# haowenz/chromap

Hardware: AMD Instinct MI355X
Metric: M paired reads mapped/s (ATAC preset, GRCh38 index) (higher is better)
Workload: dtype u64

## Files before the change

chromap_amd/csrc/cm_api.hip:

```cpp
#include <hip/hip_runtime.h>
#include <math.h>
#include <stdio.h>
#include <stdlib.h>
#include <string.h>

#include <string>
#include <vector>

#include "../../include/chromap_amd.h"
#include "cm_barcode_translate.h"
#include "cm_ctx.h"
#include "cm_kernels.h"
#include "cm_classes.h"
#include "cm_summary.h"
#include "cm_coop.h"
#include <chrono>
#include <mutex>
#include "cm_mapq_tables.h"

static thread_local std::string g_last_error;

static bool cm_debug_pool() { static const bool on = getenv("CM_DEBUG_POOL") != nullptr; return on; }
static thread_local std::string t_last_error;
void cm_set_error(cmgpu_ctx *ctx, const std::string &msg) {
// ... 68 lines not shown
    c->opt.exchange_overlap = value ? 1 : 0;
  } else if (n == "lanes") {
    if (value < 1 || value > 8) { cm_set_error(c, "lanes: 1..8"); return CMGPU_EINVAL; }
    c->opt.lanes = (int)value;
  } else if (n == "first_read_id") {
    if (value < 0 || value > 0xffffffffll) { cm_set_error(c, "first_read_id: 0..2^32-1"); return CMGPU_EINVAL; }
    c->first_read_id = (uint32_t)value;
  } else if (n == "heavy_mid_max") {
    c->opt.heavy_mid = (int)value;
  } else if (n == "heavy_last") {
    c->opt.heavy_last = (int)value;
  } else if (n == "probe_table_shift") {
    if (value < 0 || value > 4) { cm_set_error(c, "probe_table_shift: 0..4"); return CMGPU_EINVAL; }
    return cm_build_fast_table(c, (int)value);
  } else if (n == "long_read_fused") {
    c->opt.long_fused = value ? 1 : 0;
  } else if (n == "sam_format_group") {
    if (value != 8 && value != 16 && value != 64) { cm_set_error(c, "sam_format_group: 8, 16 or 64"); return CMGPU_EINVAL; }
    c->opt.sam_group = (int)value;
  } else if (n == "verify_planes") {
    c->opt.planes = value ? 1 : 0;
  } else if (n == "speculative_sizes") {
    c->opt.spec = value ? 1 : 0;
    if (value < 0) { c->cls_seen = 0; memset(c->cls_age, 0, sizeof(c->cls_age)); }
  } else if (n == "debug_candidate_capacity") {
    if (value > 0 && cm_ensure_candidate_arrays(c, (uint64_t)value)) { cm_set_error(c, "out of device memory (candidates)"); return CMGPU_ENOMEM; }
    c->pred_m_ok = value > 0; c->m_cap = (uint64_t)value; c->pred_n = 0xffffffffu;
  } else if (n == "coop_profile") {
    if (value) { if (c->coop_prof.ensure(64 * 8)) return CMGPU_ENOMEM; CM_HIPCHECK(c, hipMemset(c->coop_prof.p, 0, 64 * 8)); } else c->coop_prof.release();
  } else if (n == "coop_run_table") {
    c->opt.coop_rb = (int)value;
  } else if (n == "coop") {
    c->opt.coop = (int)value;
  } else if (n == "generic_kernels") {
    c->opt.generic_kernels = value ? 1 : 0;
  } else if (n == "item_limit") {
    c->opt.item_limit = value > 0 ? (uint64_t)value : 0xfffffff0ull;
  } else {
    cm_set_error(c, "unknown option " + n);
    return CMGPU_EINVAL;
  }
  return CMGPU_OK;
}

extern "C" int cmgpu_get_option(const cmgpu_ctx *c, const char *name, int64_t *value) {
  if (!c || !name || !value) return CMGPU_EINVAL;
  const std::string n(name);
  if (n == "probe_lookups_per_lane") *value = c->opt.probe_variant & 15;
  else if (n == "probe_pair_prefetch") *value = (c->opt.probe_variant & 16) ? 1 : 0;
  else if (n == "mm_chunks") *value = c->opt.mm_chunks;
  else if (n == "h2d_copy_blocks") *value = c->opt.h2d_kernel;
  else if (n == "d2h_copy_blocks") *value = c->opt.d2h_kernel;
  else if (n == "prep_kernel") *value = c->opt.prep_kernel;
  else if (n == "prep_tile_reads") *value = c->opt.prep_tile_reads;
  else if (n == "item_limit") *value = (int64_t)c->opt.item_limit;
  else if (n == "lanes") *value = c->opt.lanes;
  else if (n == "coop") *value = c->opt.coop;
  else if (n == "generic_kernels") *value = c->opt.generic_kernels;
  else if (n == "alloc_us") *value = (int64_t)(c->alloc_seconds * 1e6);
  else if (n == "alloc_draw_us") *value = (int64_t)(c->alloc_draw_seconds * 1e6);
  else if (n.rfind("coop_profile_", 0) == 0) {
    const int k = atoi(n.c_str() + 13);
    unsigned long long v = 0;
    if (k < 0 || k > 63 || !c->coop_prof.p || hipMemcpy(&v, (const unsigned long long *)c->coop_prof.p + k, 8, hipMemcpyDeviceToHost) != hipSuccess) return CMGPU_EINVAL;
    *value = (int64_t)v;
  }
  else if (n == "probe_table_buckets") *value = c->fmask ? (int64_t)c->fmask + 1 : (int64_t)c->bmask + 1;
  else return CMGPU_EINVAL;
  return CMGPU_OK;
}

extern "C" const char *cmgpu_last_error(const cmgpu_ctx *ctx) { return ctx ? ctx->err.c_str() : g_last_error.c_str(); }

__global__ void k_repack(const uint32_t *__restrict__ flags, const uint64_t *__restrict__ keys,
                         const uint64_t *__restrict__ vals, uint64_t *__restrict__ bkt, uint32_t i0, uint32_t n) {
  const uint32_t j = blockIdx.x * 256 + threadIdx.x;
  if (j >= n) return;
  const uint32_t i = i0 + j;
  const uint32_t f = (flags[i >> 4] >> ((i & 0xfU) << 1)) & 3u;
  uint64_t k = keys[j], v = vals[j];
  if (f & 2u) { k = CM_EMPTY_KEY; v = 0; }
  else if (f & 1u) { k = CM_DELETED_KEY; v = 0; }
  bkt[2 * (uint64_t)i] = k;
  bkt[2 * (uint64_t)i + 1] = v;
}

__global__ __launch_bounds__(256) void k_rehash(const uint64_t *__restrict__ src, uint64_t n_src, uint64_t *__restrict__ dst, uint32_t mask) {
  const uint64_t i = (uint64_t)blockIdx.x * 256 + threadIdx.x;
  if (i >= n_src) return;
  const uint64_t key = src[2 * i], val = src[2 * i + 1];
  if (key == CM_EMPTY_KEY || key == CM_DELETED_KEY) return;
// ... 538 lines not shown
  d.goff = (const uint32_t *)c->goff.p; d.n_seq = c->n_seq;
  d.ref_pl = c->ref_pl_words && c->opt.planes ? (const CmPlRec *)c->ref_planes.p + CM_PL_LEAD : nullptr; d.ref_pl_words = c->ref_pl_words;
  d.p = c->p; d.p.single = c->single ? 1 : 0;
  d.mq.len_coef = (const double *)c->len_coef.p; d.mq.nsec_break = (const uint32_t *)c->nsec_break.p; d.mq.n_break = c->n_break;
  d.n_pairs = hi - lo; d.first_read_id = c->first_read_id + lo;
  d.rb0 = (const uint8_t *)c->rb0.p; d.rb1 = (const uint8_t *)c->rb1.p;
  d.ro0 = (const uint32_t *)c->ro0.p + lo; d.ro1 = (const uint32_t *)c->ro1.p + lo;
#define PTR(f, T) d.f = (T *)c->f.p;
  PTR(rlen, uint32_t) PTR(mm_cnt, uint32_t)
  PTR(mm_off, uint32_t) PTR(mm_hash, uint64_t) PTR(mm_ps, uint32_t) PTR(pr_val, uint64_t) PTR(pr_kind, uint8_t)
  PTR(hit_tot, uint32_t) PTR(hit_off, uint32_t) PTR(round2, uint8_t) PTR(rep_cnt, uint32_t) PTR(rep_len, uint32_t)
  PTR(hbuf, uint64_t) PTR(hcnt, uint8_t) PTR(n_pos_hit, uint32_t) PTR(ncp, uint32_t) PTR(ncn, uint32_t)
  PTR(aug, uint8_t) PTR(res_neg, int32_t) PTR(res_pos, int32_t) PTR(resc_n, uint32_t) PTR(resc_p, uint32_t)
  PTR(m_tot, uint32_t) PTR(m_off, uint32_t) PTR(mbuf, uint64_t) PTR(mcnt, uint8_t) PTR(mcp, uint32_t) PTR(mcn, uint32_t)
  PTR(force0, uint8_t) PTR(fbuf, uint64_t) PTR(fcnt, uint8_t) PTR(fcp, uint32_t) PTR(fcn, uint32_t) PTR(alive, uint8_t)
  PTR(dpos, uint64_t) PTR(derr, int16_t) PTR(dsplit, uint32_t) PTR(nv, uint32_t) PTR(v_off, uint32_t) PTR(v_err, int16_t) PTR(v_end, int16_t) PTR(ndp, uint32_t) PTR(ndn, uint32_t)
  PTR(min_err, int32_t) PTR(second_err, int32_t) PTR(n_best, int32_t) PTR(n_second, int32_t)
  PTR(pe_min, int32_t) PTR(pe_second, int32_t) PTR(pe_nbest, int32_t) PTR(pe_nsecond, int32_t)
  PTR(pe_first, uint32_t) PTR(pe_i1, uint32_t) PTR(pe_i2, uint32_t) PTR(pe_choice, uint32_t)
  PTR(stats, unsigned long long) PTR(srt_cnt, uint32_t) PTR(srt_list, uint32_t) PTR(hv_cnt, uint32_t) PTR(hv_list, uint32_t) PTR(rs_cnt, uint32_t) PTR(rs_list, uint32_t)
#undef PTR
  d.rec = (uint8_t *)c->rec.p + (size_t)lo * 24 * cm_rec_per_pair(c);
  d.rec_ok = (uint8_t *)c->rec_ok.p + (size_t)lo * cm_rec_per_pair(c);
  d.hv_stride = 2 * (hi - lo) + 1;
  d.perm_reads = c->use_perm ? (const uint32_t *)c->perm_reads.p : nullptr; d.perm_pairs = c->use_perm ? (const uint32_t *)c->perm_pairs.p : nullptr;
  d.coop_slab = (uint8_t *)c->coop_slab.p; d.coop_slab_cap = CM_SLAB_CAP; d.coop_slab_blocks = CM_SLAB_BLOCKS;
  d.cls_mask = c->cls_all || !c->opt.spec ? ~0ull : c->cls_seen;
  d.prof = (unsigned long long *)c->coop_prof.p;
  d.rs_pool = (uint64_t *)c->rs_pool.p; d.rs_pool_cap = c->rs_pool.p ? c->rs_pool_cap : 0u; d.rs_pool_off = (uint32_t *)c->rs_pool_off.p;
  d.abort = (const unsigned long long *)c->stats.p + CM_ST_ABORT;
  d.coop_rb = c->opt.coop_rb > 0 ? (uint32_t)c->opt.coop_rb : 0u;
  d.wq_dynamic = ((uint32_t)c->opt.coop >> 16) & 1u;
  d.generic_kernels = c->opt.generic_kernels ? 1u : 0u;
  if (c->has_rank) {
    d.rid_rank = (const uint32_t *)c->rid_rank.p;
    d.ref_off = (const uint64_t *)c->ref_off_r.p;
    d.ref_len = (const uint32_t *)c->ref_len_r.p;
  }
  if (c->has_pairs_rank) d.pairs_rank = (const uint32_t *)c->pairs_rank.p;
  if (c->has_barcodes) {
    d.bcb = (const uint8_t *)c->bcb.p; d.bcq = (const uint8_t *)c->bcq.p; d.bco = (const uint32_t *)c->bco.p + lo;
    d.wl = (const uint64_t *)c->wl.p; d.wl_mask = c->wl_mask; d.wl_num_sample = (double)c->wl_num_sample;
    d.pow10_tab = (const double *)c->pow10_tab.p;
    d.bc_key = c->bc_key.p ? (uint64_t *)c->bc_key.p + lo : nullptr; d.bc_ok = c->bc_ok.p ? (uint8_t *)c->bc_ok.p + lo : nullptr;
  }
}
static inline void mark(cmgpu_ctx *c, const char *name) {
  if (c->n_ev < CM_MAX_EVENTS) {
    (void)hipEventRecord(c->ev[c->n_ev], c->stream);
    c->ev_name[c->n_ev] = name;
    ++c->n_ev;
  }
}
static int scan_with_total(cmgpu_ctx *c, const uint32_t *in, uint32_t *out, uint32_t n, unsigned long long *total, bool wait = true) {
  hipStream_t s = c->stream;
  unsigned long long *acc = (unsigned long long *)c->stats.p + CM_ST_TOTAL;
  CM_HIPCHECK(c, hipMemsetAsync(acc, 0, 8, s));
  cm_launch_k_sum_u32(in, n, acc, s);
  cm_scan_u32(in, out, n, (uint32_t *)c->scan_tmp.p, s);
  CM_HIPCHECK(c, hipMemcpyAsync(total, acc, 8, hipMemcpyDeviceToHost, s));
  if (wait) CM_HIPCHECK(c, cm_stream_sync(s));
  return CMGPU_OK;
}
#define CM_RC_SPLIT (-100)
#define CM_RC_AGAIN_ALL_CLASSES (-101)
#define CM_RC_AGAIN_EXACT_SIZES (-102)
// ... 1202 lines not shown
```

chromap_amd/csrc/cm_ctx.h:

```cpp
#ifndef CM_CTX_H_
#define CM_CTX_H_
#include <hip/hip_runtime.h>

#include <string>
#include <thread>
#include <vector>

#include "../../include/chromap_amd.h"
#include "../../include/chromap_amd_debug.h"
#include "cm_types.h"

#define CM_MAX_EVENTS 32
#define CM_MAX_W_HOST 32

struct DevBuf {
  void *p = nullptr;
  size_t cap = 0;
  bool owned = true;
  int ensure(size_t bytes);
  void release();
};

struct CmTmpBuf : private DevBuf {
  using DevBuf::p;
// ... 67 lines not shown
  unsigned long long *h_matrix = nullptr;
  hipStream_t stream = nullptr;
  hipEvent_t ev_part = nullptr, ev_payload = nullptr;
  bool payload_pending = false;
  uint64_t sent_total = 0, recv_total = 0, steps = 0;
  uint64_t owned_by[64] = {};
};

#define CM_BATCH_SLOTS 8
struct CmBatchSlot {
  DevBuf rb0, rb1, ro0, ro1;
  uint32_t n_pairs = 0, first_read_id = 0, max_read_len = 1;
  size_t bases0 = 0, bases1 = 0;
};

struct CmOptions {
  int long_fused = 1;
  int planes = 1;
  int sam_group = 8;
  int d2h_kernel = 0;
  int h2d_kernel = 0;
  int probe_variant = 1;
  int mm_chunks = CM_MM_CHUNKS;
  int prep_tile_reads = 32;
  int prep_kernel = 0;
  uint64_t item_limit = 0xfffffff0ull;
  int exchange_overlap = 0;
  int s3b_cap = 0;
  int lanes = 1;
  int heavy_mid = 0;
  int heavy_max[3] = {0, 0, 0};
  int heavy_last = 0;
  int spec = 1;
  int generic_kernels = 0;
  int coop_rb = 0;
  int coop = 0xff;
};

struct cmgpu_ctx {
  CmOptions opt;
  int device = 0;
  hipStream_t stream = nullptr;
  hipStream_t stream2 = nullptr;
  hipStream_t stream_pack = nullptr;
  hipEvent_t chunk_ev[CM_MM_CHUNKS + 1] = {};
  std::string err;
  cmgpu_params hp;
  CmParams p;
  DevBuf bkt, occ, ref, ref_off, ref_len, len_coef, nsec_break;
  uint32_t bmask = 0, n_occ = 0, n_seq = 0;
  DevBuf bkt_fast, coop_prof;
  uint32_t fmask = 0;
  DevBuf ref_planes, read_planes;
  DevBuf mm_stage;
  uint64_t ref_pl_words = 0;
  int n_break = 0;
  uint64_t ref_bytes = 0;
  std::vector<uint64_t> h_ref_off;
  std::vector<uint32_t> h_ref_len;
  uint32_t n_pairs = 0, first_read_id = 0;
  size_t bases0 = 0, bases1 = 0;
  uint32_t max_read_len = 1;
  DevBuf rb0, rb1, ro0, ro1;
  DevBuf st_rb0, st_rb1, st_ro0, st_ro1, st_bcb, st_bcq, st_bco;
  DevBuf rlen, scratch_a, scratch_b , mm_cnt, mm_off, mm_hash, mm_ps, pr_val, pr_kind;
  DevBuf hit_tot, hit_off, round2, rep_cnt, rep_len, hbuf, hcnt, n_pos_hit, ncp, ncn;
// ... 155 lines not shown
```

chromap_amd/csrc/cm_kernels.hip:

```cpp
#include <hip/hip_runtime.h>
#include <stdio.h>
#include <string.h>
#include <cstring>
#include <atomic>
#include <map>
#include <mutex>
#include <type_traits>
#include <utility>
#include <rocprim/rocprim.hpp>

#include "cm_kernels.h"
#include "cm_stages.h"
#include "cm_classes.h"
#include "cm_coop.h"

#define CM_BLOCK 256

#define CM_ITEM_KERNEL(kname, fn, perm)                                      \
  __global__ __launch_bounds__(CM_BLOCK) void kname(CmDev d, uint32_t n) {   \
    if (d.abort && *d.abort) return;                                         \
    const uint32_t i = blockIdx.x * CM_BLOCK + threadIdx.x;                  \
    if (i < n) fn(d, d.perm ? d.perm[i] : i);                                \
  }

// ... 294 lines not shown
__global__ __launch_bounds__(CM_BLOCK) void k_s3a_count(CmDev d, uint32_t n) {
  const uint32_t i = blockIdx.x * CM_BLOCK + threadIdx.x;
  uint32_t tot = 0;
  if (i < n) {
    cm_s3a_count(d, i);
    tot = d.hit_tot[i];
  }
  const uint32_t cls = cm_hit_class(d, tot);
  __shared__ uint32_t sh_cnt[8], sh_base[8];
  if (threadIdx.x < 8) sh_cnt[threadIdx.x] = 0;
  __syncthreads();
  const uint32_t lane = threadIdx.x & 63u;
  const uint32_t ids[8] = {CM_L_HIT_WAVE, CM_L_HIT_B256A, CM_L_HIT_B256B, CM_L_HIT_SLAB, CM_L_HIT_G16, CM_L_HIT_B512, CM_L_HIT_WAVE_SMALL, CM_L_HIT_B1024};
  uint32_t slot = 0, mine = 8;
#pragma unroll
  for (uint32_t q = 0; q < 8; ++q) {
    const unsigned long long m = __ballot(cls == ids[q]);
    if (m == 0) continue;
    uint32_t base = 0;
    if (lane == (uint32_t)(__ffsll((long long)m) - 1)) base = atomicAdd(&sh_cnt[q], (uint32_t)__popcll(m));
    base = __shfl(base, __ffsll((long long)m) - 1, 64);
    if (cls == ids[q]) { slot = base + (uint32_t)__popcll(m & ((1ull << lane) - 1ull)); mine = q; }
  }
  __syncthreads();
  if (threadIdx.x < 8 && sh_cnt[threadIdx.x]) sh_base[threadIdx.x] = atomicAdd(cm_list_cnt(d, ids[threadIdx.x]), sh_cnt[threadIdx.x]);
  __syncthreads();
  if (mine < 8) cm_list(d, ids[mine])[sh_base[mine] + slot] = i;
}
__global__ __launch_bounds__(CM_BLOCK) void k_s3b_candidates(CmDev d, uint32_t n, uint32_t cap) {
  uint64_t *sh_h = reinterpret_cast<uint64_t *>(cm_lds);
  uint8_t *sh_c = cm_lds + (size_t)cap * blockDim.x * 8;
  const uint32_t i = blockIdx.x * blockDim.x + threadIdx.x;
  if (i < n && d.hit_tot[i] <= cap) cm_s3b_candidates_lds(d, i, sh_h + threadIdx.x, sh_c + threadIdx.x, cap, blockDim.x);
}

template <int G>
__device__ __forceinline__ void cm_group_sync() {
  if (G <= 64) {
    __builtin_amdgcn_fence(__ATOMIC_RELEASE, "workgroup");
    __builtin_amdgcn_wave_barrier();
    __builtin_amdgcn_fence(__ATOMIC_ACQUIRE, "workgroup");
  } else {
    __syncthreads();
  }
}

template <int G>
__global__ __launch_bounds__(CM_BLOCK) void k_s3b_heavy(CmDev d, const uint32_t *__restrict__ list, uint32_t n_list, uint32_t P,
                                                        const uint32_t *__restrict__ n_list_dev) {
  constexpr int GPB = CM_BLOCK / G;
  const uint32_t grp = threadIdx.x / G, t = threadIdx.x % G;
  if (n_list_dev) n_list = *n_list_dev;
  uint64_t *S = reinterpret_cast<uint64_t *>(cm_lds) + (size_t)grp * P;
  uint16_t *oc = reinterpret_cast<uint16_t *>(cm_lds + (size_t)GPB * P * 8) + (size_t)grp * P;
  uint32_t *ctr = reinterpret_cast<uint32_t *>(cm_lds + (size_t)GPB * P * 10) + (size_t)grp * (G + 8);
  for (uint32_t gid = blockIdx.x * GPB + grp; gid < n_list; gid += gridDim.x * GPB) {
  const uint32_t r = list[gid];
  const uint32_t tot = d.hit_tot[r];
  const uint32_t b = d.mm_off[r], n = d.mm_cnt[r];
  const uint32_t maxf = d.round2[r] ? (uint32_t)d.p.f1 : (uint32_t)d.p.f0;
  const uint64_t SB = 1ull << 63;
  uint32_t P2 = 2;
  while (P2 < tot) P2 <<= 1;
  if (t == 0) { ctr[0] = 0; ctr[1] = 0; }
  for (uint32_t i = tot + t; i < P2; i += G) S[i] = ~0ull;
  cm_group_sync<G>();
// ... 934 lines not shown
  for (int off = 32; off > 0; off >>= 1) {
    steps += __shfl_down(steps, off, 64);
    hit += __shfl_down(hit, off, 64);
  }
  if ((threadIdx.x & 63) == 0) { sh_s[threadIdx.x >> 6] = steps; sh_h[threadIdx.x >> 6] = hit; }
  __syncthreads();
  if (threadIdx.x == 0) {
    uint32_t a = 0, c = 0;
    for (int j = 0; j < CM_BLOCK / 64; ++j) { a += sh_s[j]; c += sh_h[j]; }
    block_partials[blockIdx.x] = make_uint2(a, c);
  }
}

template <int U, bool PAIR>
__global__ __launch_bounds__(CM_BLOCK) void k_probe(const uint64_t *__restrict__ bkt, uint32_t bmask,
                                                     const uint64_t *__restrict__ hash, uint64_t *__restrict__ val,
                                                     uint8_t *__restrict__ kind, uint32_t n,
                                                     uint2 *__restrict__ block_partials) {
  uint32_t steps = 0, hit = 0;
  cm_probe_lanes<U, PAIR>(bkt, bmask, hash, val, kind, 0ull, (unsigned long long)n, (unsigned long long)blockIdx.x * (U * CM_BLOCK), &steps, &hit);
  if (block_partials) cm_probe_account(steps, hit, block_partials);
}

template <int U, bool PAIR>
__global__ __launch_bounds__(CM_BLOCK) void k_probe_range(const uint64_t *__restrict__ bkt, uint32_t bmask,
                                                           const uint64_t *__restrict__ hash, uint64_t *__restrict__ val,
                                                           uint8_t *__restrict__ kind, const unsigned long long *__restrict__ range,
                                                           uint32_t cap, uint2 *__restrict__ block_partials) {
  const unsigned long long lo = range[0];
  unsigned long long hi = range[1];
  if (hi > cap) hi = cap;
  uint32_t steps = 0, hit = 0;
  const unsigned long long tile0 = lo + (unsigned long long)blockIdx.x * (U * CM_BLOCK);
  if (tile0 < hi) cm_probe_lanes<U, PAIR>(bkt, bmask, hash, val, kind, lo, hi, tile0, &steps, &hit);
  cm_probe_account(steps, hit, block_partials);
}

__global__ __launch_bounds__(CM_BLOCK) void k_probe_reduce(const uint2 *__restrict__ partials, uint32_t n_blocks,
                                                            unsigned long long *__restrict__ counters) {
  unsigned long long a = 0, c = 0;
  for (uint32_t i = blockIdx.x * CM_BLOCK + threadIdx.x; i < n_blocks; i += gridDim.x * CM_BLOCK) { a += partials[i].x; c += partials[i].y; }
  for (int off = 32; off > 0; off >>= 1) {
    a += __shfl_down(a, off, 64);
    c += __shfl_down(c, off, 64);
  }
  __shared__ unsigned long long sa[CM_BLOCK / 64], sc[CM_BLOCK / 64];
  if ((threadIdx.x & 63) == 0) { sa[threadIdx.x >> 6] = a; sc[threadIdx.x >> 6] = c; }
  __syncthreads();
  if (threadIdx.x == 0) {
    for (int j = 1; j < CM_BLOCK / 64; ++j) { a += sa[j]; c += sc[j]; }
    if (a) atomicAdd(&counters[0], a);
    if (c) atomicAdd(&counters[1], c);
  }
}

#define CM_NSTAT 8
#define CM_STATS_BLOCKS 2048u
__global__ __launch_bounds__(CM_BLOCK) void k_stats(CmDev d, uint32_t n, unsigned long long *__restrict__ partials) {
  unsigned long long v[CM_NSTAT] = {0, 0, 0, 0, 0, 0, 0, 0};
  for (uint32_t pair = blockIdx.x * CM_BLOCK + threadIdx.x; pair < n; pair += gridDim.x * CM_BLOCK) {
    const uint32_t r1 = 2 * pair, r2 = r1 + 1;
    if (d.alive[pair]) {
      v[0] += d.fcp[r1] + d.fcn[r1] + d.fcp[r2] + d.fcn[r2];
      const uint32_t nd1 = d.ndp[r1] + d.ndn[r1], nd2 = d.ndp[r2] + d.ndn[r2];
      const unsigned long long per = d.p.single ? 1ull : 2ull;
      if (nd1 > 0 && (d.p.single || nd2 > 0)) {
        const int nb = d.pe_nbest[pair];
// ... 261 lines not shown
        uint32_t *sl = cm_list(d, CM_L_HIT_SERIAL), *sc = cm_list_cnt(d, CM_L_HIT_SERIAL);
        hipLaunchKernelGGL((k_s3b_coop<1024, false>), dim3(blocks), dim3(1024), lds, s, d, lst(CM_L_HIT_SLAB), n_cls[CM_L_HIT_SLAB], d.hv_max[3], MM, RB, sl, sc, 1u);
        hipLaunchKernelGGL(k_s3b_serial, dim3(64), dim3(64), 0, s, d, (const uint32_t *)sl, 0u, (const uint32_t *)sc);
        rest[CM_L_HIT_SLAB] = 0;
      }
    }
    if (any_coop) {
      const uint32_t P = pow2(d.hv_big > d.hv_max[3] ? d.hv_big : d.hv_max[3]);
      hipLaunchKernelGGL(k_s3b_heavy<CM_BLOCK>, dim3(512), dim3(CM_BLOCK), (size_t)P * 10 + (CM_BLOCK + 8) * 4, s, d, (const uint32_t *)fb_list, 0u, P, (const uint32_t *)fb_cnt);
    }
  }
  for (uint32_t c : {(uint32_t)CM_L_HIT_WAVE_SMALL, (uint32_t)CM_L_HIT_WAVE}) {
    if (!rest[c]) continue;
    const uint32_t P = pow2(d.hv_max[0]), gpb = CM_BLOCK / 64;
    hipLaunchKernelGGL(k_s3b_heavy<64>, dim3((rest[c] + gpb - 1) / gpb), dim3(CM_BLOCK), (size_t)gpb * P * 10 + gpb * (64 + 8) * 4, s, d, lst(c), rest[c], P, (const uint32_t *)nullptr);
  }
  const uint32_t blk[4][2] = {{CM_L_HIT_B256A, CM_P_HV1}, {CM_L_HIT_B256B, CM_P_HV2}, {CM_L_HIT_B512, CM_P_HV3}, {CM_L_HIT_B1024, CM_P_HV_BIG}};
  for (int q = 0; q < 4; ++q) {
    const uint32_t c = blk[q][0];
    if (!rest[c]) continue;
    const uint32_t P = pow2(cm_class_size(d, blk[q][1]));
    hipLaunchKernelGGL(k_s3b_heavy<CM_BLOCK>, dim3(rest[c]), dim3(CM_BLOCK), (size_t)P * 10 + (CM_BLOCK + 8) * 4, s, d, lst(c), rest[c], P, (const uint32_t *)nullptr);
  }
  if (rest[CM_L_HIT_SLAB]) hipLaunchKernelGGL(k_s3b_serial, dim3((rest[CM_L_HIT_SLAB] + 63) / 64), dim3(64), 0, s, d, lst(CM_L_HIT_SLAB), rest[CM_L_HIT_SLAB], (const uint32_t *)nullptr);
  if (rest[CM_L_HIT_G16]) {
    const uint32_t P = pow2(d.hv_mid), gpb = CM_BLOCK / 16;
    hipLaunchKernelGGL(k_s3b_heavy<16>, dim3((rest[CM_L_HIT_G16] + gpb - 1) / gpb), dim3(CM_BLOCK), (size_t)gpb * P * 10 + gpb * (16 + 8) * 4, s, d, lst(CM_L_HIT_G16), rest[CM_L_HIT_G16], P, (const uint32_t *)nullptr);
  }
}
void cm_launch_k_s3b_candidates(const CmDev &d, uint32_t n, uint32_t max_read_len, hipStream_t s) {
  if (!n) return;
  const uint32_t cap = d.s3b_cap;
  (void)max_read_len;
  uint32_t threads = 256;
  while (threads > 64 && (size_t)cap * threads * 9 > 36 * 1024 + 1024) threads >>= 1;
  hipLaunchKernelGGL(k_s3b_candidates, dim3((n + threads - 1) / threads), dim3(threads), (size_t)cap * threads * 9, s, d, n, cap);
}
uint32_t cm_rescue_seg_cap(uint32_t n_reads) { return ((n_reads + CM_BLOCK - 1) / CM_BLOCK / CM_RS_SEGS + 1) * CM_BLOCK; }
static inline bool cm_mode_pe(const CmDev &d) { return !d.p.split && !d.p.single && !d.generic_kernels; }
#define CM_LAUNCH_MODE(kname, ...) do { if (cm_mode_pe(d)) hipLaunchKernelGGL(kname<CmModePe>, __VA_ARGS__); else hipLaunchKernelGGL(kname<CmModeAny>, __VA_ARGS__); } while (0)
void cm_launch_k_s4a_rescue_count(const CmDev &d, uint32_t n, hipStream_t s, bool coop) {
  if (n) CM_LAUNCH_MODE(k_s4a_rescue_count, grid_for(n), dim3(CM_BLOCK), 0, s, d, n, cm_rescue_seg_cap(n), coop ? 1u : 0u);
}
static inline uint32_t rescue_wave_blocks(uint32_t n_reads) {
  uint32_t b = n_reads / 512 + 64;
  return b > 8192u ? 8192u : b;
}
static inline dim3 rescue_list_grid(uint32_t n_reads) {
  uint32_t b = n_reads / 64 / CM_RS_SEGS / 4 + 1;
  if (b > 256u) b = 256u;
  return dim3(b, CM_RS_SEGS);
}
void cm_launch_k_s4a_rescue_list(const CmDev &d, uint32_t n_reads, hipStream_t s, bool coop) {
  if (!n_reads) return;
  hipLaunchKernelGGL(k_s4a_rescue_list, rescue_list_grid(n_reads), dim3(64), 0, s, d, cm_rescue_seg_cap(n_reads), coop ? 1u : 0u);
  if ((coop) && cm_cls_on(d, CM_L_SEARCH_WAVE)) {
    hipLaunchKernelGGL(k_s4a_rescue_wave<true>, dim3(rescue_wave_blocks(n_reads)), dim3(64), 0, s, d);
    hipLaunchKernelGGL(k_s4a_rescue_wave<false>, dim3(rescue_wave_blocks(n_reads)), dim3(64), 0, s, d);
  }
}
static const CmClassRow cm_s4b_rows[] = {
  {CM_L_RS_WAVE, 64, 128, 2, 2048, 2048, CM_P_HV0, 0},
  {CM_L_RS_B256A, 256, 256, 1, 2048, 2048, CM_P_HV1, CM_P_HV0},
  {CM_L_RS_B256B, 256, 256, 1, 2048, 2048, CM_P_HV2, CM_P_HV1},
  {CM_L_RS_B512, 512, 512, 1, 2048, 512, CM_P_RS_MAX3, CM_P_HV2},
  {CM_L_RS_B1024, 1024, 1024, 1, 2048, 256, CM_P_RS_BIG, CM_P_RS_MAX3},
// ... 257 lines not shown
```

chromap_amd/csrc/cm_stages.h:

```cpp
#ifndef CM_STAGES_H_
#define CM_STAGES_H_

#include "cm_types.h"

struct CmModeAny {
  static constexpr bool kPe = false;
  static CM_HD bool split(const CmDev &d) { return d.p.split != 0; }
  static CM_HD bool single(const CmDev &d) { return d.p.single != 0; }
};
struct CmModePe {
  static constexpr bool kPe = true;
  static CM_HD bool split(const CmDev &) { return false; }
  static CM_HD bool single(const CmDev &) { return false; }
};

CM_HD uint32_t cm_c2u(uint8_t c) {
  const uint32_t u = c & 0xDFu;
  const uint32_t x = (u >> 1) & 3u;
  const uint32_t o = u - 0x41u;
  const bool acgt = o < 20u && ((0x80045u >> (o & 31u)) & 1u);
  return acgt ? x ^ (x >> 1) : 4u;
}
CM_HD uint8_t cm_negchar(uint8_t c) {
  const uint32_t v = 3u ^ cm_c2u(c);
// ... 1083 lines not shown
  }
  cm_sort_u64_strided(h, np, st);
  cm_sort_u64_strided(h + (size_t)np * st, nn, st);
  const bool use_high = d.round2[r] && np > 0 && nn > 0;
  int req = (int)n - (int)d.rep_cnt[r];
  req = req > 1 ? req : 1;
  req = req > d.p.min_seeds ? d.p.min_seeds : req;
  if (use_high) req = d.p.min_seeds;
  *np_out = np;
  *ncp_out = cm_sweep_strided(h, hc, np, d.p.e, req, n, st);
  *ncn_out = cm_sweep_strided(h + (size_t)np * st, hc + (size_t)np * st, nn, d.p.e, req, n, st);
}

CM_HD void cm_s3b_candidates_lds(const CmDev &d, uint32_t r, uint64_t *lds_h, uint8_t *lds_c, uint32_t lds_cap,
                                 uint32_t lds_stride) {
  const uint32_t tot = d.hit_tot[r];
  d.ncp[r] = 0; d.ncn[r] = 0; d.n_pos_hit[r] = 0;
  if (tot == 0) return;
  uint64_t *h = d.hbuf + d.hit_off[r];
  uint8_t *hc = d.hcnt + d.hit_off[r];
  uint32_t np, ncp, ncn;
  if (lds_h && tot <= lds_cap) {
    cm_s3b_core(d, r, lds_h, lds_c, lds_stride, &np, &ncp, &ncn);
    for (uint32_t i = 0; i < ncp; ++i) { h[i] = lds_h[i * lds_stride]; hc[i] = lds_c[i * lds_stride]; }
    for (uint32_t i = 0; i < ncn; ++i) { h[np + i] = lds_h[(np + i) * lds_stride]; hc[np + i] = lds_c[(np + i) * lds_stride]; }
  } else {
    cm_s3b_core(d, r, h, hc, 1, &np, &ncp, &ncn);
  }
  d.n_pos_hit[r] = np;
  d.ncp[r] = ncp;
  d.ncn[r] = ncn;
}
CM_HD void cm_s3b_candidates(const CmDev &d, uint32_t r) { cm_s3b_candidates_lds(d, r, nullptr, nullptr, 0, 1); }

CM_HD bool cm_rescue_bails(const CmDev &d, int max_count, int best_num, uint32_t mn) {
  return best_num >= 300 || mn > (uint32_t)d.p.f0 || (max_count <= d.p.min_seeds && best_num >= 200);
}
CM_HD uint32_t cm_rescue_minimizer(const CmDev &d, int strand, const uint64_t *mp, const uint8_t *mc, uint32_t mn, int max_count,
                                   uint8_t kind, uint64_t val, uint32_t ps, uint64_t *out, unsigned long long *reads_out) {
  if (kind == CM_PR_MISS) return 0;
  const uint32_t search_range = 2u * (uint32_t)d.p.max_insert;
  uint32_t cnt = 0;
  unsigned long long reads = 0;
  bool same;
  if (kind == CM_PR_SINGLE) {
    const uint64_t cp = cm_cand_from_hit(val, ps, d.p.k, &same);
    if ((same && strand == 0) || (!same && strand == 1)) { if (out) out[cnt] = cp; ++cnt; }
    return cnt;
  }
  const uint32_t off = (uint32_t)(val >> 32), nocc = (uint32_t)val;
  const uint64_t *o = d.occ + off;
  int32_t prev_l = 0;
  uint32_t ci = 0;
  bool have = false;
  uint64_t ws = 0, we = 0;
  for (;;) {
    bool emit = false;
    uint64_t es = 0, ee = 0;
    while (ci < mn) {
      if (mc[ci] != max_count) { ++ci; continue; }
      const uint64_t pos = mp[ci];
      const uint64_t s = pos < search_range ? 0 : pos - search_range;
      const uint64_t en = pos + search_range;
      ++ci;
      if (!have) { ws = s; we = en; have = true; continue; }
      if (we < s) { es = ws; ee = we; emit = true; ws = s; we = en; break; }
// ... 594 lines not shown
  for (uint32_t j0 = 0; j0 < 32; j0 += 8) {
    uint64_t v = j0 < n ? cm_load8(bytes + j0) : 0;
    for (uint32_t j = j0; j < j0 + 8; ++j, v >>= 8) {
      const uint32_t u = j < n ? cm_c2u((uint8_t)v) : 4u;
      q0 |= (u & 1u) << j; q1 |= ((u >> 1) & 1u) << j; qn |= (u >> 2) << j;
      qc |= (j < n && (uint8_t)v >= 'a' && (uint8_t)v <= 'z' ? 1u : 0u) << j;
    }
  }
  *p0 = q0; *p1 = q1; *pn = qn;
  if (pc) *pc = qc;
}
CM_HD uint32_t cm_read_pl_stride(uint32_t W) { return (6u * W + 3u) & ~3u; }
CM_HD uint32_t *cm_read_pl_of(const CmDev &d, uint32_t r) { return d.read_pl + (size_t)r * cm_read_pl_stride(d.read_pl_w); }
CM_HD void cm_pack_read_planes_any(const CmDev &d, uint32_t r) {
  const uint32_t W = d.read_pl_w, L = d.rlen[r];
  if (L == 0) return;
  uint32_t *f = cm_read_pl_of(d, r), *v = f + 3 * (size_t)W;
  const uint8_t *read = cm_read_ptr(d, r);
  const uint32_t nw = (L + 31) >> 5;
  for (uint32_t w = 0; w < nw; ++w) cm_pack_planes32(read + 32 * w, L - 32 * w, f + w, f + W + w, f + 2 * W + w);
  for (uint32_t w = 0; w < nw; ++w) {
    const int lo = (int)L - 32 * (int)w - 32;
    uint32_t F[3];
    for (int q = 0; q < 3; ++q) {
      const uint32_t *src = f + (size_t)q * W;
      if (lo >= 0) {
        const uint32_t a = (uint32_t)lo >> 5, sh = (uint32_t)lo & 31u;
        F[q] = cm_funnel32(src[a], a + 1 < nw ? src[a + 1] : 0u, sh);
      } else F[q] = src[0] << (uint32_t)(-lo);
    }
    v[w] = ~cm_brev32(F[0]); v[W + w] = ~cm_brev32(F[1]); v[2 * W + w] = cm_brev32(F[2]);
  }
}
template <int W>
CM_HD void cm_pack_read_planes_w(const CmDev &d, uint32_t r) {
  const uint32_t L = d.rlen[r];
  if (L == 0) return;
  const uint8_t *read = cm_read_ptr(d, r);
  uint32_t o[6 * W];
  const uintptr_t ra = reinterpret_cast<uintptr_t>(read);
  const uint32_t sh8 = (uint32_t)(ra & 7) * 8;
  const uint64_t *ap = reinterpret_cast<const uint64_t *>(ra & ~(uintptr_t)7);
  uint64_t wv[4 * W + 1];
#pragma unroll
  for (int q = 0; q <= 4 * W; ++q) wv[q] = (uint32_t)q * 8u < (sh8 >> 3) + L ? ap[q] : 0ull;
#pragma unroll
  for (int w = 0; w < W; ++w) {
    uint32_t q0 = 0, q1 = 0, qn = 0;
#pragma unroll
    for (int k = 0; k < 4; ++k) {
      uint64_t v = sh8 ? (wv[4 * w + k] >> sh8) | (wv[4 * w + k + 1] << (64u - sh8)) : wv[4 * w + k];
#pragma unroll
      for (int b = 0; b < 8; ++b, v >>= 8) {
        const uint32_t j = (uint32_t)(8 * k + b);
        const uint32_t u = 32u * (uint32_t)w + j < L ? cm_c2u((uint8_t)v) : 4u;
        q0 |= (u & 1u) << j; q1 |= ((u >> 1) & 1u) << j; qn |= (u >> 2) << j;
      }
    }
    o[w] = q0; o[W + w] = q1; o[2 * W + w] = qn;
  }
#pragma unroll
  for (int q = 0; q < 3; ++q) {
    uint32_t *v = o + 3 * W + q * W;
#pragma unroll
    for (int w = 0; w < W; ++w) v[w] = cm_brev32(o[q * W + (W - 1 - w)]);
    uint32_t s = 32u * W - L;
    while (s >= 32) {
#pragma unroll
      for (int w = 0; w + 1 < W; ++w) v[w] = v[w + 1];
      v[W - 1] = 0;
      s -= 32;
    }
    if (s) {
#pragma unroll
      for (int w = 0; w < W; ++w) v[w] = (v[w] >> s) | (w + 1 < W ? v[w + 1] << (32u - s) : 0u);
    }
    if (q < 2) {
#pragma unroll
      for (int w = 0; w < W; ++w) v[w] = ~v[w];
    }
  }
  uint32_t *dst = cm_read_pl_of(d, r);
  struct alignas(16) Q { uint32_t a, b, c, e; };
#pragma unroll
  for (int i = 0; i < 6 * W; i += 4) {
    Q x = {o[i], i + 1 < 6 * W ? o[i + 1] : 0u, i + 2 < 6 * W ? o[i + 2] : 0u, i + 3 < 6 * W ? o[i + 3] : 0u};
    *reinterpret_cast<Q *>(dst + i) = x;
  }
}
CM_HD void cm_pack_read_planes(const CmDev &d, uint32_t r) {
  switch (d.read_pl_w) {
// ... 1320 lines not shown
```

chromap_amd/csrc/cm_types.h:

```cpp
#ifndef CM_TYPES_H_
#define CM_TYPES_H_

#include <stddef.h>
#include <stdint.h>

#if defined(__HIPCC__)
#include <hip/hip_runtime.h>
#define CM_HD __host__ __device__ __forceinline__
#define CM_D __device__ __forceinline__
#else
#define CM_HD inline
#define CM_D inline
#endif

#define CM_EMPTY_KEY 0xFFFFFFFFFFFFFFFFull
#define CM_DELETED_KEY 0xFFFFFFFFFFFFFFFEull

#define CM_PR_MISS 0
#define CM_PR_SINGLE 1
#define CM_PR_MULTI 2
#define CM_V_INVALID 0x7fff
#define CM_MM_CHUNKS 8
enum CmList : uint32_t {
  CM_L_HIT_WAVE = 0, CM_L_HIT_B256A = 1, CM_L_HIT_B256B = 2, CM_L_HIT_SLAB = 3, CM_L_HIT_G16 = 4, CM_L_HIT_DECLINED = 5, CM_L_RS_WAVE = 6, CM_L_RS_B256A = 7,
// ... 78 lines not shown
  uint32_t *mm_ps;
  uint64_t *pr_val;
  uint8_t *pr_kind;
  uint32_t *hit_tot;
  uint32_t *hit_off;
  uint8_t *round2;
  uint32_t *rep_cnt;
  uint32_t *rep_len;
  uint64_t *hbuf;
  uint8_t *hcnt;
  uint32_t *n_pos_hit;
  uint32_t *ncp, *ncn;
  const uint32_t *perm_reads, *perm_pairs;
  uint32_t *hv_cnt, *hv_list;
  uint32_t *rs_cnt, *rs_list;
  uint32_t *srt_cnt, *srt_list;
  uint32_t hv_big, rs_max3, rs_big;
  unsigned long long cls_mask;
  uint32_t s4c_pbig, s5c_pblock;
  uint32_t hv_stride, s3b_cap, hv_max[4];
  uint8_t *coop_slab;
  uint32_t coop_slab_cap;
  uint32_t coop_slab_blocks;
  const unsigned long long *abort;
  uint64_t *rs_pool;
  uint32_t rs_pool_cap;
  uint32_t *rs_pool_off;
  uint32_t wq_dynamic;
  unsigned long long *prof;
  uint32_t mm_cap;
  uint32_t coop_rb;
  uint32_t hv_sub;
  uint32_t generic_kernels;
  uint32_t hv_mid;
  uint8_t *aug;
  int32_t *res_neg;
  int32_t *res_pos;
  uint32_t *resc_n;
  uint32_t *resc_p;
  uint32_t *m_tot;
  uint32_t *m_off;
  uint64_t *mbuf;
  uint8_t *mcnt;
  uint32_t *mcp, *mcn;
  uint8_t *force0;
  uint64_t *fbuf;
  uint8_t *fcnt;
  uint32_t *fcp, *fcn;
  uint8_t *alive;
  uint64_t *dpos;
  int16_t *derr;
  uint32_t *dsplit;
  uint32_t *ndp, *ndn;
  uint32_t *nv;
  uint32_t *v_off;
  int16_t *v_err;
  int16_t *v_end;
  int32_t *min_err, *second_err, *n_best, *n_second;
  int32_t *pe_min, *pe_second, *pe_nbest, *pe_nsecond;
  uint32_t *pe_first;
  uint32_t *pe_i1, *pe_i2;
  uint32_t *pe_choice;
  uint8_t *rec;
  uint8_t *rec_ok;
  const uint32_t *rid_rank;
  const uint32_t *pairs_rank;
// ... 32 lines not shown
```

Baseline: 557.9.

## Add sorting-network short-candidate kernel, SWAR read plane packing, early-exit probe blocks

Adds a specialised stage-3b kernel for reads with at most 16 hits. It stages hits in static LDS columns, sorts them in registers with a bitonic-style network, and emits candidates in one unrolled pass instead of the generic dynamic-LDS path. Separately, read-plane packing now uses SWAR bit tricks to convert 8 bases at a time instead of a per-byte loop. Empty probe blocks now zero their partials and return early. Together these aim to cut per-read sorting and packing cost, at the risk of subtle mismatches with the generic candidate logic.

After: 578.8, median of 6. 3.8% higher.

```diff
diff --git a/chromap_amd/csrc/cm_api.hip b/chromap_amd/csrc/cm_api.hip
--- a/chromap_amd/csrc/cm_api.hip
+++ b/chromap_amd/csrc/cm_api.hip
@@ -124,6 +124,8 @@
     c->opt.coop_rb = (int)value;
   } else if (n == "coop") {
     c->opt.coop = (int)value;
+  } else if (n == "s3b_short") {
+    c->opt.s3b_short = value ? 1 : 0;
   } else if (n == "generic_kernels") {
     c->opt.generic_kernels = value ? 1 : 0;
   } else if (n == "item_limit") {
@@ -149,6 +151,7 @@
   else if (n == "lanes") *value = c->opt.lanes;
   else if (n == "coop") *value = c->opt.coop;
   else if (n == "generic_kernels") *value = c->opt.generic_kernels;
+  else if (n == "s3b_short") *value = c->opt.s3b_short;
   else if (n == "alloc_us") *value = (int64_t)(c->alloc_seconds * 1e6);
   else if (n == "alloc_draw_us") *value = (int64_t)(c->alloc_draw_seconds * 1e6);
   else if (n.rfind("coop_profile_", 0) == 0) {
@@ -753,6 +756,7 @@
   d.coop_rb = c->opt.coop_rb > 0 ? (uint32_t)c->opt.coop_rb : 0u;
   d.wq_dynamic = ((uint32_t)c->opt.coop >> 16) & 1u;
   d.generic_kernels = c->opt.generic_kernels ? 1u : 0u;
+  d.s3b_short = c->opt.s3b_short ? 1u : 0u;
   if (c->has_rank) {
     d.rid_rank = (const uint32_t *)c->rid_rank.p;
     d.ref_off = (const uint64_t *)c->ref_off_r.p;
diff --git a/chromap_amd/csrc/cm_ctx.h b/chromap_amd/csrc/cm_ctx.h
--- a/chromap_amd/csrc/cm_ctx.h
+++ b/chromap_amd/csrc/cm_ctx.h
@@ -123,6 +123,7 @@
   int heavy_max[3] = {0, 0, 0};
   int heavy_last = 0;
   int spec = 1;
+  int s3b_short = 1;
   int generic_kernels = 0;
   int coop_rb = 0;
   int coop = 0xff;
diff --git a/chromap_amd/csrc/cm_kernels.hip b/chromap_amd/csrc/cm_kernels.hip
--- a/chromap_amd/csrc/cm_kernels.hip
+++ b/chromap_amd/csrc/cm_kernels.hip
@@ -350,6 +350,13 @@
   uint8_t *sh_c = cm_lds + (size_t)cap * blockDim.x * 8;
   const uint32_t i = blockIdx.x * blockDim.x + threadIdx.x;
   if (i < n && d.hit_tot[i] <= cap) cm_s3b_candidates_lds(d, i, sh_h + threadIdx.x, sh_c + threadIdx.x, cap, blockDim.x);
+}
+
+template <int BLOCK>
+__global__ __launch_bounds__(BLOCK) void k_s3b_short(CmDev d, uint32_t n) {
+  __shared__ uint64_t sh_h[CM_S3S_CAP * BLOCK];
+  const uint32_t i = blockIdx.x * BLOCK + threadIdx.x;
+  if (i < n && d.hit_tot[i] <= CM_S3S_CAP) cm_s3b_short<BLOCK>(d, i, sh_h, threadIdx.x);
 }
 
 template <int G>
@@ -1350,7 +1357,11 @@
   if (hi > cap) hi = cap;
   uint32_t steps = 0, hit = 0;
   const unsigned long long tile0 = lo + (unsigned long long)blockIdx.x * (U * CM_BLOCK);
-  if (tile0 < hi) cm_probe_lanes<U, PAIR>(bkt, bmask, hash, val, kind, lo, hi, tile0, &steps, &hit);
+  if (tile0 >= hi) {
+    if (threadIdx.x == 0) block_partials[blockIdx.x] = make_uint2(0u, 0u);
+    return;
+  }
+  cm_probe_lanes<U, PAIR>(bkt, bmask, hash, val, kind, lo, hi, tile0, &steps, &hit);
   cm_probe_account(steps, hit, block_partials);
 }
 
@@ -1678,6 +1689,10 @@
   if (!n) return;
   const uint32_t cap = d.s3b_cap;
   (void)max_read_len;
+  if (cap == CM_S3S_CAP && d.s3b_short && d.n_seq < 0x80000000u) {
+    hipLaunchKernelGGL(k_s3b_short<CM_BLOCK>, dim3((n + CM_BLOCK - 1) / CM_BLOCK), dim3(CM_BLOCK), 0, s, d, n);
+    return;
+  }
   uint32_t threads = 256;
   while (threads > 64 && (size_t)cap * threads * 9 > 36 * 1024 + 1024) threads >>= 1;
   hipLaunchKernelGGL(k_s3b_candidates, dim3((n + threads - 1) / threads), dim3(threads), (size_t)cap * threads * 9, s, d, n, cap);
diff --git a/chromap_amd/csrc/cm_stages.h b/chromap_amd/csrc/cm_stages.h
--- a/chromap_amd/csrc/cm_stages.h
+++ b/chromap_amd/csrc/cm_stages.h
@@ -1139,6 +1139,121 @@
   d.ncn[r] = ncn;
 }
 CM_HD void cm_s3b_candidates(const CmDev &d, uint32_t r) { cm_s3b_candidates_lds(d, r, nullptr, nullptr, 0, 1); }
+
+#define CM_S3S_CAP 16
+CM_HD void cm_cmpx_u64(uint64_t &a, uint64_t &b) {
+  const bool sw = b < a;
+  const uint64_t lo = sw ? b : a, hi = sw ? a : b;
+  a = lo; b = hi;
+}
+CM_HD void cm_sort16_network(uint64_t (&a)[CM_S3S_CAP]) {
+#pragma unroll
+  for (int p = 1; p < CM_S3S_CAP; p <<= 1) {
+#pragma unroll
+    for (int k = p; k >= 1; k >>= 1) {
+#pragma unroll
+      for (int j = k % p; j + k < CM_S3S_CAP; j += 2 * k) {
+#pragma unroll
+        for (int i = 0; i < k; ++i) {
+          if (i + j + k < CM_S3S_CAP && (i + j) / (2 * p) == (i + j + k) / (2 * p)) cm_cmpx_u64(a[i + j], a[i + j + k]);
+        }
+      }
+    }
+  }
+}
+template <int BLOCK>
+CM_HD void cm_s3b_short_put(uint64_t *col, uint32_t *cnt, uint32_t *np, uint64_t ref_hit, uint32_t ps, int k) {
+  bool same;
+  const uint64_t cp = cm_cand_from_hit(ref_hit, ps, k, &same);
+  col[((*cnt)++) * (uint32_t)BLOCK] = same ? cp : cp | (1ull << 63);
+  *np += same ? 1u : 0u;
+}
+template <int BLOCK>
+CM_HD void cm_s3b_short_lists(const CmDev &d, uint32_t r, uint32_t tot, uint64_t *S, uint32_t t, uint32_t *np_out, uint32_t *ncp_out,
+                              uint32_t *ncn_out) {
+  static_assert(BLOCK > 0 && (BLOCK & (BLOCK - 1)) == 0, "the slot index is a shift");
+  const uint32_t b = d.mm_off[r], n = d.mm_cnt[r];
+  const uint32_t maxf = d.round2[r] ? (uint32_t)d.p.f1 : (uint32_t)d.p.f0;
+  const uint64_t SB = 1ull << 63;
+  uint64_t *col = S + t;
+  uint32_t cnt = 0, np = 0;
+  for (uint32_t i0 = 0; i0 < n; i0 += CM_S3B_GROUP) {
+    uint8_t kind[CM_S3B_GROUP];
+    uint64_t val[CM_S3B_GROUP], first[CM_S3B_GROUP];
+    uint32_t ps[CM_S3B_GROUP];
+#pragma unroll
+    for (int q = 0; q < CM_S3B_GROUP; ++q) {
+      const bool in = i0 + q < n;
+      kind[q] = in ? d.pr_kind[b + i0 + q] : (uint8_t)CM_PR_MISS;
+      val[q] = in ? d.pr_val[b + i0 + q] : 0;
+      ps[q] = in ? d.mm_ps[b + i0 + q] : 0;
+    }
+    uint32_t len[CM_S3B_GROUP];
+#pragma unroll
+    for (int q = 0; q < CM_S3B_GROUP; ++q) {
+      const uint32_t nocc = (uint32_t)val[q];
+      const bool single = kind[q] == CM_PR_SINGLE;
+      const bool run = kind[q] != CM_PR_MISS && !single && nocc < maxf && nocc > 0;
+      len[q] = single ? 1u : run ? nocc : 0u;
+      first[q] = run ? d.occ[(uint32_t)(val[q] >> 32)] : val[q];
+    }
+#pragma unroll
+    for (int q = 0; q < CM_S3B_GROUP; ++q) {
+      if (len[q] == 0) continue;
+      cm_s3b_short_put<BLOCK>(col, &cnt, &np, first[q], ps[q], d.p.k);
+      const uint64_t *o = d.occ + (uint32_t)(val[q] >> 32);
+      for (uint32_t oi = 1; oi < len[q]; ++oi) cm_s3b_short_put<BLOCK>(col, &cnt, &np, o[oi], ps[q], d.p.k);
+    }
+  }
+  uint64_t a[CM_S3S_CAP];
+#pragma unroll
+  for (int i = 0; i < CM_S3S_CAP; ++i) a[i] = (uint32_t)i < tot ? col[(uint32_t)i * (uint32_t)BLOCK] : ~0ull;
+  cm_sort16_network(a);
+  const bool use_high = d.round2[r] && np > 0 && np < tot;
+  int req = (int)n - (int)d.rep_cnt[r];
+  req = req > 1 ? req : 1;
+  req = req > d.p.min_seeds ? d.p.min_seeds : req;
+  if (use_high) req = d.p.min_seeds;
+  const uint32_t e = (uint32_t)d.p.e;
+  uint64_t *h = d.hbuf + d.hit_off[r];
+  uint8_t *hc = d.hcnt + d.hit_off[r];
+  uint32_t out_p = 0, out_n = 0;
+  int mcount = 1, equal = 1, best_equal = 1;
+  uint64_t prev_hit = a[0], best_local = a[0];
+#pragma unroll
+  for (int pi = 1; pi <= CM_S3S_CAP; ++pi) {
+    if ((uint32_t)pi <= tot) {
+      const uint64_t x = pi < CM_S3S_CAP ? a[pi < CM_S3S_CAP ? pi : 0] : ~0ull;
+      const bool brk = (uint32_t)(x >> 32) != (uint32_t)(prev_hit >> 32) || (uint32_t)x > (uint32_t)prev_hit + e ||
+                       ((uint32_t)mcount >= n && (uint32_t)x > (uint32_t)best_local + e);
+      if (brk && mcount >= req) {
+        const bool neg = (best_local >> 63) != 0;
+        const uint32_t at = neg ? np + out_n : out_p;
+        h[at] = best_local & ~SB;
+        hc[at] = (uint8_t)best_equal;
+        out_n += neg ? 1u : 0u; out_p += neg ? 0u : 1u;
+      }
+      const bool eq_best = x == best_local, eq_prev = x == prev_hit;
+      const int equal1 = eq_best || eq_prev ? equal + 1 : 1;
+      const bool take_prev = !eq_best && eq_prev && equal1 > best_equal;
+      best_equal = brk ? 1 : eq_best ? best_equal + 1 : take_prev ? equal1 : best_equal;
+      best_local = brk ? x : take_prev ? prev_hit : best_local;
+      equal = brk ? 1 : equal1;
+      mcount = brk ? 1 : mcount + 1;
+      prev_hit = x;
+    }
+  }
+  *np_out = np; *ncp_out = out_p; *ncn_out = out_n;
+}
+template <int BLOCK>
+CM_HD void cm_s3b_short(const CmDev &d, uint32_t r, uint64_t *S, uint32_t t) {
+  const uint32_t tot = d.hit_tot[r];
+  uint32_t np = 0, ncp = 0, ncn = 0;
+  if (tot) cm_s3b_short_lists<BLOCK>(d, r, tot, S, t, &np, &ncp, &ncn);
+  d.n_pos_hit[r] = np;
+  d.ncp[r] = ncp;
+  d.ncn[r] = ncn;
+}
 
 CM_HD bool cm_rescue_bails(const CmDev &d, int max_count, int best_num, uint32_t mn) {
   return best_num >= 300 || mn > (uint32_t)d.p.f0 || (max_count <= d.p.min_seeds && best_num >= 200);
@@ -1799,6 +1914,24 @@
     v[w] = ~cm_brev32(F[0]); v[W + w] = ~cm_brev32(F[1]); v[2 * W + w] = cm_brev32(F[2]);
   }
 }
+CM_HD void cm_pack4_bits(uint32_t w, uint32_t *b0, uint32_t *b1, uint32_t *bn) {
+  const uint32_t x = (w >> 1) & 0x03030303u;
+  const uint32_t code = x ^ ((x >> 1) & 0x01010101u);
+  const uint32_t is_t = (x >> 1) & ~x & 0x01010101u;
+  const uint32_t diff = ((w & 0xD9D9D9D9u) ^ 0x41414141u) ^ (is_t | (is_t << 4));
+  const uint32_t nz = ((diff & 0x7F7F7F7Fu) + 0x7F7F7F7Fu) | diff;
+  *b0 = code & 0x01010101u; *b1 = (code >> 1) & 0x01010101u; *bn = (nz >> 7) & 0x01010101u;
+}
+CM_HD uint32_t cm_fold8(uint32_t u) {
+  u |= u >> 7;
+  return (u | (u >> 14)) & 0xFFu;
+}
+CM_HD void cm_pack8_planes(uint32_t a, uint32_t b, uint32_t *p0, uint32_t *p1, uint32_t *pn) {
+  uint32_t a0, a1, an, c0, c1, cn;
+  cm_pack4_bits(a, &a0, &a1, &an);
+  cm_pack4_bits(b, &c0, &c1, &cn);
+  *p0 = cm_fold8(a0 | (c0 << 4)); *p1 = cm_fold8(a1 | (c1 << 4)); *pn = cm_fold8(an | (cn << 4));
+}
 template <int W>
 CM_HD void cm_pack_read_planes_w(const CmDev &d, uint32_t r) {
   const uint32_t L = d.rlen[r];
@@ -1816,14 +1949,14 @@
     uint32_t q0 = 0, q1 = 0, qn = 0;
 #pragma unroll
     for (int k = 0; k < 4; ++k) {
-      uint64_t v = sh8 ? (wv[4 * w + k] >> sh8) | (wv[4 * w + k + 1] << (64u - sh8)) : wv[4 * w + k];
-#pragma unroll
-      for (int b = 0; b < 8; ++b, v >>= 8) {
-        const uint32_t j = (uint32_t)(8 * k + b);
-        const uint32_t u = 32u * (uint32_t)w + j < L ? cm_c2u((uint8_t)v) : 4u;
-        q0 |= (u & 1u) << j; q1 |= ((u >> 1) & 1u) << j; qn |= (u >> 2) << j;
-      }
-    }
+      const uint64_t v = sh8 ? (wv[4 * w + k] >> sh8) | (wv[4 * w + k + 1] << (64u - sh8)) : wv[4 * w + k];
+      uint32_t p0, p1, pn;
+      cm_pack8_planes((uint32_t)v, (uint32_t)(v >> 32), &p0, &p1, &pn);
+      q0 |= p0 << (8 * k); q1 |= p1 << (8 * k); qn |= pn << (8 * k);
+    }
+    const uint32_t left = L > 32u * (uint32_t)w ? L - 32u * (uint32_t)w : 0u;
+    if (left < 32u) qn |= ~0u << left;
+    q0 &= ~qn; q1 &= ~qn;
     o[w] = q0; o[W + w] = q1; o[2 * W + w] = qn;
   }
 #pragma unroll
diff --git a/chromap_amd/csrc/cm_types.h b/chromap_amd/csrc/cm_types.h
--- a/chromap_amd/csrc/cm_types.h
+++ b/chromap_amd/csrc/cm_types.h
@@ -134,6 +134,7 @@
   uint32_t coop_rb;
   uint32_t hv_sub;
   uint32_t generic_kernels;
+  uint32_t s3b_short;
   uint32_t hv_mid;
   uint8_t *aug;
   int32_t *res_neg;
```
